# samxuxiang/BrepGen

Measured on NVIDIA H100. Metric: B-reps/sec (1000-step ABC cascade), higher is better.
Workload: dtype f16 x f16 -> f32 (wgmma; split hi+lo weights on in/out-proj; fp32 residual/LN/softmax)

## Files before the change

brepgen_b200/csrc/gemm.cu:

```cuda
#include <stdlib.h>

#include "bg_internal.h"
#include "gemm_epilogue.cuh"
#include "ptx.cuh"

namespace bg {

namespace {

constexpr int BM = 128;
constexpr int BK = 64;

template <int BN>
struct Cfg {
  static constexpr int STAGES = (BN == 256) ? 4 : 6;
  static constexpr int A_BYTES = BM * BK * 2;
  static constexpr int B_BYTES = BN * BK * 2;
  static constexpr int STAGE_BYTES = A_BYTES + B_BYTES;
  static constexpr int BAR_BYTES = 256;
  static constexpr int SMEM_BYTES = STAGES * STAGE_BYTES + BAR_BYTES + 1024;
};

template <int BN>
__device__ __forceinline__ void wgmma_tile_k16(float (&acc)[BN / 2], uint64_t a, uint64_t b, uint32_t accumulate) {
  if constexpr (BN == 256) wgmma_m64n256k16_ss(acc, a, b, accumulate);
  else wgmma_m64n128k16_ss(acc, a, b, accumulate);
}

template <int BN>
__global__ void __launch_bounds__(384, 1)
gemm_f16_kernel(const __grid_constant__ CUtensorMap tmA, const __grid_constant__ CUtensorMap tmB, const GemmParams p_in) {
  const GemmParams p = gemm_resolve(p_in);
  using C = Cfg<BN>;
  extern __shared__ uint8_t smem_raw[];
  uint8_t* smem = reinterpret_cast<uint8_t*>((reinterpret_cast<uintptr_t>(smem_raw) + 1023) & ~uintptr_t(1023));
  uint64_t* full = reinterpret_cast<uint64_t*>(smem + C::STAGES * C::STAGE_BYTES);
  uint64_t* empty = full + C::STAGES;

  const int warp = threadIdx.x >> 5;
  const int lane = threadIdx.x & 31;
  const int wg = threadIdx.x >> 7;

  if (threadIdx.x == 0) {
    tma_prefetch_desc(&tmA);
    tma_prefetch_desc(&tmB);
    for (int i = 0; i < C::STAGES; ++i) {
      mbar_init(&full[i], 1);
      mbar_init(&empty[i], 256);
    }
    fence_barrier_init();
  }
  __syncthreads();

  const int num_m = (p.M + BM - 1) / BM;
  const int num_n = p.N / BN;
  const int num_tiles = num_m * num_n;
  const int num_k = p.K / BK;

  if (wg == 0) {
    setmaxnreg_dec<40>();
    if (warp == 0 && elect_one()) {
      int stage = 0;
      uint32_t phase = 0;
      for (int tile = blockIdx.x; tile < num_tiles; tile += gridDim.x) {
        const int m_blk = tile / num_n, n_blk = tile % num_n;
        const int nk = (n_blk * BN < p.n_short) ? p.k_short / BK : num_k;
        gemm_prefetch_resid<BM, BN>(p, m_blk * BM, n_blk * BN);
        for (int kb = 0; kb < nk; ++kb) {
          mbar_wait(&empty[stage], phase ^ 1);
          uint8_t* sA = smem + stage * C::STAGE_BYTES;
          uint8_t* sB = sA + C::A_BYTES;
          mbar_arrive_expect_tx(&full[stage], C::STAGE_BYTES);
          if (p.conv_taps) {
            int c0, x, y, n;
            conv_coords(p, kb, m_blk * BM, c0, x, y, n);
            tma_load_4d(sA, &tmA, &full[stage], c0, x, y, n);
          } else {
            const int ka = p.a_kwrap ? (kb * BK) % p.a_kwrap : kb * BK;
            tma_load_2d(sA, &tmA, &full[stage], ka, m_blk * BM);
          }
          tma_load_2d(sB, &tmB, &full[stage], kb * BK, n_blk * BN);
          if (++stage == C::STAGES) { stage = 0; phase ^= 1; }
        }
      }
    }
  } else {
    setmaxnreg_inc<232>();
    const int half = wg - 1;
    float acc[BN / 2];
    int stage = 0;
    uint32_t phase = 0;
    for (int tile = blockIdx.x; tile < num_tiles; tile += gridDim.x) {
      const int m_blk = tile / num_n, n_blk = tile % num_n;
      const int nk = (n_blk * BN < p.n_short) ? p.k_short / BK : num_k;
      int prev = -1;
      for (int kb = 0; kb < nk; ++kb) {
        mbar_wait(&full[stage], phase);
        const uint32_t a_addr = smem_u32(smem + stage * C::STAGE_BYTES) + half * 64 * 128;
        const uint32_t b_addr = smem_u32(smem + stage * C::STAGE_BYTES + C::A_BYTES);
        wgmma_fence_operand(acc);
        wgmma_fence();
#pragma unroll
        for (int k = 0; k < BK / 16; ++k)
          wgmma_tile_k16<BN>(acc, make_sw128_desc(a_addr + k * 32), make_sw128_desc(b_addr + k * 32), (kb | k) != 0 ? 1u : 0u);
        wgmma_commit();
        wgmma_fence_operand(acc);
        wgmma_wait<1>();
        if (prev >= 0) mbar_arrive(&empty[prev]);
        prev = stage;
        if (++stage == C::STAGES) { stage = 0; phase ^= 1; }
      }
      wgmma_wait<0>();
      wgmma_fence_operand(acc);
      mbar_arrive(&empty[prev]);
      gemm_epilogue_regs<BN>(p, acc, m_blk * BM + half * 64, n_blk * BN, warp & 3, lane);
    }
  }
}

template <int BN>
int launch_bn(cudaStream_t st, const CUtensorMap& tmA, const CUtensorMap& tmB, const GemmParams& p) {
  using C = Cfg<BN>;
  BG_TRY(ensure_dynamic_smem(reinterpret_cast<const void*>(&gemm_f16_kernel<BN>), C::SMEM_BYTES));
  const int num_tiles = ((p.M + BM - 1) / BM) * (p.N / BN);
  const int grid = num_tiles < num_sms() ? num_tiles : num_sms();
  gemm_f16_kernel<BN><<<grid, 384, C::SMEM_BYTES, st>>>(tmA, tmB, p);
  return check_launch("gemm_f16_kernel launch");
}

namespace pp {
constexpr int BN = 128;
constexpr int STAGES = 5;
constexpr int STAGE_BYTES = (BM + BN) * BK * 2;
constexpr int BOX_BYTES = BM * 128;
constexpr int STAGING_BYTES = BM * BN * 4;
constexpr int BAR_BYTES = 256;
constexpr int SMEM_BYTES = STAGES * STAGE_BYTES + STAGING_BYTES + BAR_BYTES + 1024;
}

__device__ __forceinline__ void pp_advance(int& stage, uint32_t& phase, int n) {
  stage += n;
  while (stage >= pp::STAGES) { stage -= pp::STAGES; phase ^= 1; }
}

__device__ __forceinline__ void pp_arm_staging(const GemmParams& p, const CUtensorMap* tmR, uint8_t* stg, uint64_t* bar,
                                               int tile, int num_n) {
  if (p.resid) {
    const int row0 = (tile / num_n) * BM, col0 = (tile % num_n) * pp::BN;
    mbar_arrive_expect_tx(bar, pp::STAGING_BYTES);
#pragma unroll
    for (int b = 0; b < 4; ++b) tma_load_2d(stg + b * pp::BOX_BYTES, tmR, bar, col0 + 32 * b, row0);
  } else {
    mbar_arrive(bar);
  }
}

__device__ __forceinline__ void pp_epilogue_smem(const GemmParams& p, const float (&acc)[2][64], uint8_t* stg, int col0,
                                                 int warp_in_wg, int lane) {
  const int q = lane & 3;
#pragma unroll
  for (int i = 0; i < pp::BN / 8; ++i) {
    float2 b = make_float2(0.f, 0.f);
    if (p.bias) b = __ldg(reinterpret_cast<const float2*>(p.bias + col0 + 8 * i + 2 * q));
#pragma unroll
    for (int h = 0; h < 2; ++h) {
#pragma unroll
      for (int hr = 0; hr < 2; ++hr) {
        const int r = h * 64 + warp_in_wg * 16 + hr * 8 + (lane >> 2);
        float v0 = acc[h][4 * i + 2 * hr], v1 = acc[h][4 * i + 2 * hr + 1];
        if (p.bias) {
          v0 += b.x;
          v1 += b.y;
        }
        float2* d = reinterpret_cast<float2*>(stg + (i >> 2) * pp::BOX_BYTES + r * 128 +
                                              (((2 * (i & 3) + (q >> 1)) ^ (r & 7)) << 4) + 8 * (q & 1));
        if (p.resid) {
          const float2 rr = *d;
          v0 += rr.x;
          v1 += rr.y;
        }
        if (p.relu) {
          v0 = fmaxf(v0, 0.f);
          v1 = fmaxf(v1, 0.f);
        }
        *d = make_float2(v0, v1);
      }
    }
  }
}

__global__ void __launch_bounds__(384, 1)
gemm_pp_kernel(const __grid_constant__ CUtensorMap tmA, const __grid_constant__ CUtensorMap tmB,
               const __grid_constant__ CUtensorMap tmO, const __grid_constant__ CUtensorMap tmR, const GemmParams p_in) {
  const GemmParams p = gemm_resolve(p_in);
  extern __shared__ uint8_t smem_raw[];
  uint8_t* smem = reinterpret_cast<uint8_t*>((reinterpret_cast<uintptr_t>(smem_raw) + 1023) & ~uintptr_t(1023));
  uint8_t* stg = smem + pp::STAGES * pp::STAGE_BYTES;
  uint64_t* full = reinterpret_cast<uint64_t*>(stg + pp::STAGING_BYTES);
  uint64_t* empty = full + pp::STAGES;
  uint64_t* turn = empty + pp::STAGES;
  uint64_t* ready = turn + 2;

  const int warp = threadIdx.x >> 5;
  const int lane = threadIdx.x & 31;
  const int wg = threadIdx.x >> 7;

  const int num_m = (p.M + BM - 1) / BM;
  const int num_n = p.N / pp::BN;
  const int num_tiles = num_m * num_n;
  const int num_k = p.K / BK;

  if (threadIdx.x == 0) {
    tma_prefetch_desc(&tmA);
    tma_prefetch_desc(&tmB);
    tma_prefetch_desc(&tmO);
    for (int i = 0; i < pp::STAGES; ++i) {
      mbar_init(&full[i], 1);
      mbar_init(&empty[i], 128);
    }
    for (int c = 0; c < 2; ++c) {
      mbar_init(&turn[c], 128);
      mbar_init(&ready[c], 1);
    }
    fence_barrier_init();
  }
  __syncthreads();
  if (threadIdx.x == 0 && (int)blockIdx.x < num_tiles) pp_arm_staging(p, &tmR, stg, &ready[0], blockIdx.x, num_n);

  if (wg == 0) {
    setmaxnreg_dec<40>();
    if (warp == 0 && elect_one()) {
      int stage = 0;
      uint32_t phase = 0;
      for (int tile = blockIdx.x; tile < num_tiles; tile += gridDim.x) {
        const int m_blk = tile / num_n, n_blk = tile % num_n;
        const int nk = (n_blk * pp::BN < p.n_short) ? p.k_short / BK : num_k;
        for (int kb = 0; kb < nk; ++kb) {
          mbar_wait(&empty[stage], phase ^ 1);
          uint8_t* sA = smem + stage * pp::STAGE_BYTES;
          uint8_t* sB = sA + BM * BK * 2;
          mbar_arrive_expect_tx(&full[stage], pp::STAGE_BYTES);
          const int ka = p.a_kwrap ? (kb * BK) % p.a_kwrap : kb * BK;
          tma_load_2d(sA, &tmA, &full[stage], ka, m_blk * BM);
          tma_load_2d(sB, &tmB, &full[stage], kb * BK, n_blk * pp::BN);
          pp_advance(stage, phase, 1);
        }
      }
    }
  } else {
    setmaxnreg_inc<232>();
    const int c = wg - 1;
    float acc[2][64];
    int stage = 0;
    uint32_t phase = 0;
    int j = 0;
    for (int t = 0, tile = blockIdx.x; tile < num_tiles; ++t, tile += gridDim.x) {
      const int m_blk = tile / num_n, n_blk = tile % num_n;
      const int nk = (n_blk * pp::BN < p.n_short) ? p.k_short / BK : num_k;
      if ((t & 1) != c) {
        pp_advance(stage, phase, nk);
        continue;
      }
      if (t > 0) mbar_wait(&turn[c], ((t - 1) >> 1) & 1);
      int prev = -1;
      for (int kb = 0; kb < nk; ++kb) {
        mbar_wait(&full[stage], phase);
        const uint32_t a_addr = smem_u32(smem + stage * pp::STAGE_BYTES);
        const uint32_t b_addr = a_addr + BM * BK * 2;
        wgmma_fence_operand(acc[0]);
        wgmma_fence_operand(acc[1]);
        wgmma_fence();
#pragma unroll
        for (int k = 0; k < BK / 16; ++k) {
          const uint64_t bd = make_sw128_desc(b_addr + k * 32);
          wgmma_m64n128k16_ss(acc[0], make_sw128_desc(a_addr + k * 32), bd, (kb | k) != 0 ? 1u : 0u);
          wgmma_m64n128k16_ss(acc[1], make_sw128_desc(a_addr + 64 * 128 + k * 32), bd, (kb | k) != 0 ? 1u : 0u);
        }
        wgmma_commit();
        wgmma_fence_operand(acc[0]);
        wgmma_fence_operand(acc[1]);
        wgmma_wait<1>();
        if (prev >= 0) mbar_arrive(&empty[prev]);
        prev = stage;
        pp_advance(stage, phase, 1);
      }
      mbar_arrive(&turn[c ^ 1]);
      wgmma_wait<0>();
      wgmma_fence_operand(acc[0]);
      wgmma_fence_operand(acc[1]);
      mbar_arrive(&empty[prev]);

      const int row0 = m_blk * BM, col0 = n_blk * pp::BN;
      mbar_wait(&ready[c], j & 1);
      const bool leader = (threadIdx.x & 127) == 0;
      if (row0 + BM <= p.M) {
        pp_epilogue_smem(p, acc, stg, col0, warp & 3, lane);
        fence_proxy_async_shared();
        named_bar_sync(1 + c, 128);
        if (leader) {
          for (int b = 0; b < 4; ++b) tma_store_2d(&tmO, stg + b * pp::BOX_BYTES, col0 + 32 * b, row0);
          bulk_commit();
          bulk_wait_read_all();
        }
      } else {
        gemm_epilogue_regs<pp::BN>(p, acc[0], row0, col0, warp & 3, lane);
        gemm_epilogue_regs<pp::BN>(p, acc[1], row0 + 64, col0, warp & 3, lane);
      }
      if (leader && tile + (int)gridDim.x < num_tiles)
        pp_arm_staging(p, &tmR, stg, &ready[c ^ 1], tile + gridDim.x, num_n);
      ++j;
    }
  }
}

int launch_pp(cudaStream_t st, const CUtensorMap& tmA, const CUtensorMap& tmB, const CUtensorMap& tmO,
              const CUtensorMap& tmR, const GemmParams& p) {
  BG_TRY(ensure_dynamic_smem(reinterpret_cast<const void*>(&gemm_pp_kernel), pp::SMEM_BYTES));
  const int num_tiles = ((p.M + BM - 1) / BM) * (p.N / pp::BN);
  const int grid = num_tiles < num_sms() ? num_tiles : num_sms();
  gemm_pp_kernel<<<grid, 384, pp::SMEM_BYTES, st>>>(tmA, tmB, tmO, tmR, p);
  return check_launch("gemm_pp_kernel launch");
}

bool pingpong_enabled() {
  static const bool on = [] {
    const char* e = getenv("BREPGEN_B200_GEMM_PINGPONG");
    return !(e && atoi(e) == 0);
  }();
  return on;
}

}

int launch_gemm_f16(cudaStream_t st, const __half* A, int lda, const __half* W, int ldw, int M, int N, int K,
                    const GemmEpilogue& ep) {
  BG_REQUIRE(M > 0 && N > 0 && K > 0, "gemm: empty problem");
  BG_REQUIRE(K % BK == 0, "gemm: K must be a multiple of 64");
  BG_REQUIRE(N % 128 == 0, "gemm: N must be a multiple of 128");
  BG_REQUIRE(lda % 8 == 0 && ldw % 8 == 0, "gemm: operand pitch must be a multiple of 8 elements (16 B)");
  BG_REQUIRE((reinterpret_cast<uintptr_t>(A) & 15) == 0 && (reinterpret_cast<uintptr_t>(W) & 15) == 0,
             "gemm: operands must be 16-byte aligned");
  BG_REQUIRE(ep.out != nullptr && ep.ldo % 8 == 0, "gemm: output pitch must be a multiple of 8");
  BG_REQUIRE((reinterpret_cast<uintptr_t>(ep.out) & 15) == 0, "gemm: output must be 16-byte aligned");
  BG_REQUIRE(ep.resid == nullptr || (ep.ldr % 4 == 0 && !ep.out_f16 ? true : ep.ldr % 4 == 0), "gemm: resid pitch");
  BG_REQUIRE(ep.rowvec == nullptr || (ep.rows_per_vec > 0 && ep.ldv % 4 == 0), "gemm: rowvec");
  BG_REQUIRE(!ep.out_f16 || (ep.resid == nullptr && ep.rowvec == nullptr), "gemm: fp16 output supports bias / ReLU only");
  BG_REQUIRE((reinterpret_cast<uintptr_t>(ep.bias) & 7) == 0, "gemm: bias must be 8-byte aligned");
  BG_REQUIRE((reinterpret_cast<uintptr_t>(ep.resid) & 7) == 0, "gemm: resid must be 8-byte aligned");
  int bn = (N % 256 == 0) ? 256 : 128;
  if (bn == 256 && (long long)((M + BM - 1) / BM) * (N / 256) < num_sms()) bn = 128;
  const bool use_pp = pingpong_enabled() && !ep.out_f16 && ep.conv.taps == 0 && ep.rowvec == nullptr &&
                      ep.row_map == nullptr && (reinterpret_cast<uintptr_t>(ep.resid) & 15) == 0;
  if (use_pp) bn = pp::BN;
  CUtensorMap tmA, tmB;
  const int a_cols = ep.a_kwrap > 0 ? ep.a_kwrap : K;
  BG_REQUIRE(ep.a_kwrap == 0 || (ep.a_kwrap % BK == 0 && ep.a_kwrap <= K), "gemm: a_kwrap must be a multiple of 64");
  const ConvGeom& cg = ep.conv;
  if (cg.taps > 0) {
    const int hw = cg.W * cg.H;
    BG_REQUIRE(cg.C > 0 && cg.C % 64 == 0 && cg.W > 0 && cg.H > 0 && cg.N > 0 && cg.kw > 0 && cg.taps % cg.kw == 0,
               "conv gemm: bad geometry");
    BG_REQUIRE(128 % cg.W == 0 && (hw % 128 == 0 || 128 % hw == 0), "conv gemm: W * H must divide 128 or be a multiple of it");
    BG_REQUIRE(M == cg.N * hw && K == cg.terms * cg.taps * cg.C && ep.a_kwrap == 0, "conv gemm: M / K do not match the geometry");
    BG_REQUIRE(lda >= (cg.lo_plane ? 2 : 1) * cg.C, "conv gemm: channel pitch too small");
    const int box_h = hw >= 128 ? 128 / cg.W : cg.H, box_n = hw >= 128 ? 1 : 128 / hw;
    BG_TRY(make_tmap_4d_f16(&tmA, A, (uint64_t)(cg.lo_plane ? 2 : 1) * cg.C, cg.W, cg.H, cg.N, (uint64_t)lda, cg.W, box_h, box_n));
  } else {
    BG_TRY(make_tmap_2d_f16(&tmA, A, (uint64_t)M, (uint64_t)a_cols, (uint64_t)lda, BM));
  }
  BG_TRY(make_tmap_2d_f16(&tmB, W, (uint64_t)N, (uint64_t)K, (uint64_t)ldw, (uint32_t)bn));
  GemmParams p;
  p.M = M; p.N = N; p.K = K; p.a_kwrap = ep.a_kwrap; p.m_dev = ep.m_dev; p.row_map = ep.row_map;
  p.n_short = ep.n_short; p.k_short = ep.k_short;
  BG_REQUIRE(ep.n_short == 0 || (ep.n_short % 256 == 0 && ep.k_short % BK == 0 && ep.k_short > 0 && ep.k_short <= K),
             "gemm: n_short must be a multiple of 256 and k_short a multiple of 64");
  p.out = ep.out; p.ldo = ep.ldo; p.out_f16 = ep.out_f16; p.relu = ep.relu;
  p.bias = ep.bias; p.resid = ep.resid; p.ldr = ep.ldr;
  p.rowvec = ep.rowvec; p.rows_per_vec = ep.rows_per_vec; p.ldv = ep.ldv;
  p.conv_taps = cg.taps; p.conv_kw = cg.kw; p.conv_cpb = cg.C / 64; p.conv_C = cg.C; p.conv_W = cg.W; p.conv_HW = cg.W * cg.H;
  p.conv_pad_w = cg.kw / 2; p.conv_pad_h = cg.taps > 0 ? (cg.taps / cg.kw) / 2 : 0;
  p.conv_lo_term = (cg.taps > 0 && cg.lo_plane && cg.terms == 3) ? 1 : -1;
  if (use_pp) {
    CUtensorMap tmO, tmR;
    BG_TRY(make_tmap_2d_f32(&tmO, ep.out, (uint64_t)M, (uint64_t)N, (uint64_t)ep.ldo, BM, 32));
    tmR = tmO;
    if (ep.resid) BG_TRY(make_tmap_2d_f32(&tmR, ep.resid, (uint64_t)M, (uint64_t)N, (uint64_t)ep.ldr, BM, 32));
    return launch_pp(st, tmA, tmB, tmO, tmR, p);
  }
  return bn == 256 ? launch_bn<256>(st, tmA, tmB, p) : launch_bn<128>(st, tmA, tmB, p);
}

}
```

brepgen_b200/csrc/ptx.cuh:

```cuda
#pragma once
#include <cuda.h>
#include <cuda_fp16.h>
#include <cuda_runtime.h>
#include <stdint.h>

namespace bg {

__device__ __forceinline__ uint32_t smem_u32(const void* p) { return (uint32_t)__cvta_generic_to_shared(p); }

__device__ __forceinline__ bool elect_one() {
  uint32_t pred;
  asm volatile(
      "{\n\t.reg .pred P;\n\t.reg .b32 R;\n\t"
      "elect.sync R|P, 0xffffffff;\n\t"
      "selp.b32 %0, 1, 0, P;\n\t}\n"
      : "=r"(pred));
  return pred != 0;
}

__device__ __forceinline__ void mbar_init(uint64_t* bar, uint32_t count) {
  asm volatile("mbarrier.init.shared::cta.b64 [%0], %1;" ::"r"(smem_u32(bar)), "r"(count));
}
__device__ __forceinline__ void fence_barrier_init() { asm volatile("fence.mbarrier_init.release.cluster;" ::: "memory"); }
__device__ __forceinline__ void mbar_arrive(uint64_t* bar) {
  asm volatile("mbarrier.arrive.shared::cta.b64 _, [%0];" ::"r"(smem_u32(bar)) : "memory");
}
__device__ __forceinline__ void mbar_arrive_expect_tx(uint64_t* bar, uint32_t bytes) {
  asm volatile("mbarrier.arrive.expect_tx.shared::cta.b64 _, [%0], %1;" ::"r"(smem_u32(bar)), "r"(bytes) : "memory");
}
__device__ __forceinline__ bool mbar_try_wait(uint64_t* bar, uint32_t parity) {
  uint32_t ok;
  asm volatile(
      "{\n\t.reg .pred P;\n\t"
      "mbarrier.try_wait.parity.shared::cta.b64 P, [%1], %2;\n\t"
      "selp.b32 %0, 1, 0, P;\n\t}\n"
      : "=r"(ok)
      : "r"(smem_u32(bar)), "r"(parity)
      : "memory");
  return ok != 0;
}
__device__ __forceinline__ void mbar_wait(uint64_t* bar, uint32_t parity) {
  uint32_t spins = 0;
  while (!mbar_try_wait(bar, parity)) {
    if (++spins > (1u << 26)) asm volatile("trap;");
  }
}

__device__ __forceinline__ void tma_prefetch_desc(const CUtensorMap* m) {
  asm volatile("prefetch.tensormap [%0];" ::"l"(reinterpret_cast<uint64_t>(m)) : "memory");
}
__device__ __forceinline__ void tma_load_2d(void* smem_dst, const CUtensorMap* m, uint64_t* bar, int c0, int c1) {
  asm volatile(
      "cp.async.bulk.tensor.2d.shared::cluster.global.mbarrier::complete_tx::bytes [%0], [%1, {%3, %4}], [%2];"
      ::"r"(smem_u32(smem_dst)), "l"(reinterpret_cast<uint64_t>(m)), "r"(smem_u32(bar)), "r"(c0), "r"(c1)
      : "memory");
}

__device__ __forceinline__ void tma_load_4d(void* smem_dst, const CUtensorMap* m, uint64_t* bar, int c0, int c1, int c2, int c3) {
  asm volatile(
      "cp.async.bulk.tensor.4d.shared::cluster.global.mbarrier::complete_tx::bytes [%0], [%1, {%3, %4, %5, %6}], [%2];"
      ::"r"(smem_u32(smem_dst)), "l"(reinterpret_cast<uint64_t>(m)), "r"(smem_u32(bar)), "r"(c0), "r"(c1), "r"(c2), "r"(c3)
      : "memory");
}

__device__ __forceinline__ void tma_store_2d(const CUtensorMap* m, const void* smem_src, int c0, int c1) {
  asm volatile("cp.async.bulk.tensor.2d.global.shared::cta.bulk_group [%0, {%2, %3}], [%1];"
               ::"l"(reinterpret_cast<uint64_t>(m)), "r"(smem_u32(smem_src)), "r"(c0), "r"(c1)
               : "memory");
}
__device__ __forceinline__ void bulk_commit() { asm volatile("cp.async.bulk.commit_group;" ::: "memory"); }
__device__ __forceinline__ void bulk_wait_read_all() { asm volatile("cp.async.bulk.wait_group.read 0;" ::: "memory"); }
__device__ __forceinline__ void fence_proxy_async_shared() { asm volatile("fence.proxy.async.shared::cta;" ::: "memory"); }
__device__ __forceinline__ void named_bar_sync(uint32_t id, uint32_t count) {
  asm volatile("bar.sync %0, %1;" ::"r"(id), "r"(count) : "memory");
}

__device__ __forceinline__ void prefetch_l2_bulk(const void* p, uint32_t bytes) {
  asm volatile("cp.async.bulk.prefetch.L2.global [%0], %1;" ::"l"(reinterpret_cast<uint64_t>(p)), "r"(bytes) : "memory");
}

template <uint32_t N>
__device__ __forceinline__ void setmaxnreg_dec() { asm volatile("setmaxnreg.dec.sync.aligned.u32 %0;" ::"n"(N)); }
template <uint32_t N>
__device__ __forceinline__ void setmaxnreg_inc() { asm volatile("setmaxnreg.inc.sync.aligned.u32 %0;" ::"n"(N)); }

__device__ __forceinline__ uint64_t make_sw128_desc(uint32_t smem_addr, uint32_t sbo_bytes = 1024) {
  uint64_t d = 0;
  d |= (uint64_t)((smem_addr & 0x3FFFF) >> 4);
  d |= (uint64_t)1 << 16;
  d |= (uint64_t)((sbo_bytes >> 4) & 0x3FFF) << 32;
  d |= (uint64_t)1 << 62;
  return d;
}

__device__ __forceinline__ void wgmma_fence() { asm volatile("wgmma.fence.sync.aligned;" ::: "memory"); }
__device__ __forceinline__ void wgmma_commit() { asm volatile("wgmma.commit_group.sync.aligned;" ::: "memory"); }
template <int N>
__device__ __forceinline__ void wgmma_wait() { asm volatile("wgmma.wait_group.sync.aligned %0;" ::"n"(N) : "memory"); }
template <int R>
__device__ __forceinline__ void wgmma_fence_operand(float (&d)[R]) {
#pragma unroll
  for (int i = 0; i < R; ++i) asm volatile("" : "+f"(d[i])::"memory");
}

__device__ __forceinline__ void wgmma_m64n256k16_ss(float (&d)[128], uint64_t a_desc, uint64_t b_desc, uint32_t accumulate) {
  asm volatile(
      "{\n\t.reg .pred p;\n\t"
      "setp.ne.b32 p, %130, 0;\n\t"
      "wgmma.mma_async.sync.aligned.m64n256k16.f32.f16.f16 "
      "{%0, %1, %2, %3, %4, %5, %6, %7, %8, %9, %10, %11, %12, %13, %14, %15, "
      "%16, %17, %18, %19, %20, %21, %22, %23, %24, %25, %26, %27, %28, %29, %30, %31, "
      "%32, %33, %34, %35, %36, %37, %38, %39, %40, %41, %42, %43, %44, %45, %46, %47, "
      "%48, %49, %50, %51, %52, %53, %54, %55, %56, %57, %58, %59, %60, %61, %62, %63, "
      "%64, %65, %66, %67, %68, %69, %70, %71, %72, %73, %74, %75, %76, %77, %78, %79, "
      "%80, %81, %82, %83, %84, %85, %86, %87, %88, %89, %90, %91, %92, %93, %94, %95, "
      "%96, %97, %98, %99, %100, %101, %102, %103, %104, %105, %106, %107, %108, %109, %110, %111, "
      "%112, %113, %114, %115, %116, %117, %118, %119, %120, %121, %122, %123, %124, %125, %126, %127}, "
      "%128, %129, p, 1, 1, 0, 0;\n\t}\n"
      : "+f"(d[0]), "+f"(d[1]), "+f"(d[2]), "+f"(d[3]), "+f"(d[4]), "+f"(d[5]), "+f"(d[6]), "+f"(d[7]),
        "+f"(d[8]), "+f"(d[9]), "+f"(d[10]), "+f"(d[11]), "+f"(d[12]), "+f"(d[13]), "+f"(d[14]), "+f"(d[15]),
        "+f"(d[16]), "+f"(d[17]), "+f"(d[18]), "+f"(d[19]), "+f"(d[20]), "+f"(d[21]), "+f"(d[22]), "+f"(d[23]),
        "+f"(d[24]), "+f"(d[25]), "+f"(d[26]), "+f"(d[27]), "+f"(d[28]), "+f"(d[29]), "+f"(d[30]), "+f"(d[31]),
        "+f"(d[32]), "+f"(d[33]), "+f"(d[34]), "+f"(d[35]), "+f"(d[36]), "+f"(d[37]), "+f"(d[38]), "+f"(d[39]),
        "+f"(d[40]), "+f"(d[41]), "+f"(d[42]), "+f"(d[43]), "+f"(d[44]), "+f"(d[45]), "+f"(d[46]), "+f"(d[47]),
        "+f"(d[48]), "+f"(d[49]), "+f"(d[50]), "+f"(d[51]), "+f"(d[52]), "+f"(d[53]), "+f"(d[54]), "+f"(d[55]),
        "+f"(d[56]), "+f"(d[57]), "+f"(d[58]), "+f"(d[59]), "+f"(d[60]), "+f"(d[61]), "+f"(d[62]), "+f"(d[63]),
        "+f"(d[64]), "+f"(d[65]), "+f"(d[66]), "+f"(d[67]), "+f"(d[68]), "+f"(d[69]), "+f"(d[70]), "+f"(d[71]),
        "+f"(d[72]), "+f"(d[73]), "+f"(d[74]), "+f"(d[75]), "+f"(d[76]), "+f"(d[77]), "+f"(d[78]), "+f"(d[79]),
        "+f"(d[80]), "+f"(d[81]), "+f"(d[82]), "+f"(d[83]), "+f"(d[84]), "+f"(d[85]), "+f"(d[86]), "+f"(d[87]),
        "+f"(d[88]), "+f"(d[89]), "+f"(d[90]), "+f"(d[91]), "+f"(d[92]), "+f"(d[93]), "+f"(d[94]), "+f"(d[95]),
        "+f"(d[96]), "+f"(d[97]), "+f"(d[98]), "+f"(d[99]), "+f"(d[100]), "+f"(d[101]), "+f"(d[102]), "+f"(d[103]),
        "+f"(d[104]), "+f"(d[105]), "+f"(d[106]), "+f"(d[107]), "+f"(d[108]), "+f"(d[109]), "+f"(d[110]), "+f"(d[111]),
        "+f"(d[112]), "+f"(d[113]), "+f"(d[114]), "+f"(d[115]), "+f"(d[116]), "+f"(d[117]), "+f"(d[118]), "+f"(d[119]),
        "+f"(d[120]), "+f"(d[121]), "+f"(d[122]), "+f"(d[123]), "+f"(d[124]), "+f"(d[125]), "+f"(d[126]), "+f"(d[127])
      : "l"(a_desc), "l"(b_desc), "r"(accumulate));
}

__device__ __forceinline__ void wgmma_m64n128k16_ss(float (&d)[64], uint64_t a_desc, uint64_t b_desc, uint32_t accumulate) {
  asm volatile(
      "{\n\t.reg .pred p;\n\t"
      "setp.ne.b32 p, %66, 0;\n\t"
      "wgmma.mma_async.sync.aligned.m64n128k16.f32.f16.f16 "
      "{%0, %1, %2, %3, %4, %5, %6, %7, %8, %9, %10, %11, %12, %13, %14, %15, "
      "%16, %17, %18, %19, %20, %21, %22, %23, %24, %25, %26, %27, %28, %29, %30, %31, "
      "%32, %33, %34, %35, %36, %37, %38, %39, %40, %41, %42, %43, %44, %45, %46, %47, "
      "%48, %49, %50, %51, %52, %53, %54, %55, %56, %57, %58, %59, %60, %61, %62, %63}, "
      "%64, %65, p, 1, 1, 0, 0;\n\t}\n"
      : "+f"(d[0]), "+f"(d[1]), "+f"(d[2]), "+f"(d[3]), "+f"(d[4]), "+f"(d[5]), "+f"(d[6]), "+f"(d[7]),
        "+f"(d[8]), "+f"(d[9]), "+f"(d[10]), "+f"(d[11]), "+f"(d[12]), "+f"(d[13]), "+f"(d[14]), "+f"(d[15]),
        "+f"(d[16]), "+f"(d[17]), "+f"(d[18]), "+f"(d[19]), "+f"(d[20]), "+f"(d[21]), "+f"(d[22]), "+f"(d[23]),
        "+f"(d[24]), "+f"(d[25]), "+f"(d[26]), "+f"(d[27]), "+f"(d[28]), "+f"(d[29]), "+f"(d[30]), "+f"(d[31]),
        "+f"(d[32]), "+f"(d[33]), "+f"(d[34]), "+f"(d[35]), "+f"(d[36]), "+f"(d[37]), "+f"(d[38]), "+f"(d[39]),
        "+f"(d[40]), "+f"(d[41]), "+f"(d[42]), "+f"(d[43]), "+f"(d[44]), "+f"(d[45]), "+f"(d[46]), "+f"(d[47]),
        "+f"(d[48]), "+f"(d[49]), "+f"(d[50]), "+f"(d[51]), "+f"(d[52]), "+f"(d[53]), "+f"(d[54]), "+f"(d[55]),
        "+f"(d[56]), "+f"(d[57]), "+f"(d[58]), "+f"(d[59]), "+f"(d[60]), "+f"(d[61]), "+f"(d[62]), "+f"(d[63])
      : "l"(a_desc), "l"(b_desc), "r"(accumulate));
}

__device__ __forceinline__ void wgmma_m64n64k16_rs_bt(float (&d)[32], const uint32_t (&a)[4], uint64_t b_desc, uint32_t accumulate) {
  asm volatile(
      "{\n\t.reg .pred p;\n\t"
      "setp.ne.b32 p, %37, 0;\n\t"
      "wgmma.mma_async.sync.aligned.m64n64k16.f32.f16.f16 "
      "{%0, %1, %2, %3, %4, %5, %6, %7, %8, %9, %10, %11, %12, %13, %14, %15, "
      "%16, %17, %18, %19, %20, %21, %22, %23, %24, %25, %26, %27, %28, %29, %30, %31}, "
      "{%32, %33, %34, %35}, %36, p, 1, 1, 1;\n\t}\n"
      : "+f"(d[0]), "+f"(d[1]), "+f"(d[2]), "+f"(d[3]), "+f"(d[4]), "+f"(d[5]), "+f"(d[6]), "+f"(d[7]),
        "+f"(d[8]), "+f"(d[9]), "+f"(d[10]), "+f"(d[11]), "+f"(d[12]), "+f"(d[13]), "+f"(d[14]), "+f"(d[15]),
        "+f"(d[16]), "+f"(d[17]), "+f"(d[18]), "+f"(d[19]), "+f"(d[20]), "+f"(d[21]), "+f"(d[22]), "+f"(d[23]),
        "+f"(d[24]), "+f"(d[25]), "+f"(d[26]), "+f"(d[27]), "+f"(d[28]), "+f"(d[29]), "+f"(d[30]), "+f"(d[31])
      : "r"(a[0]), "r"(a[1]), "r"(a[2]), "r"(a[3]), "l"(b_desc), "r"(accumulate));
}


__device__ __forceinline__ float ex2(float x) {
  float y;
  asm("ex2.approx.ftz.f32 %0, %1;" : "=f"(y) : "f"(x));
  return y;
}

__device__ __forceinline__ uint32_t pack_half2(float a, float b) {
  __half2 h = __floats2half2_rn(a, b);
  return *reinterpret_cast<uint32_t*>(&h);
}

}
```

Baseline: 0.1905.

## Stage f16 GEMM epilogue through swizzled smem and store with TMA

For BN=256 GEMMs with f16 output and no conv taps, the epilogue now applies bias and ReLU in registers, writes packed half2 values into a 128B-swizzled shared staging buffer, and issues TMA 2D bulk stores instead of scattered register stores to global memory. Partial M tiles fall back to vectorized 16-byte copies out of the staging buffer. The aim is coalesced, asynchronous output writes that overlap with the next tile's mainloop. In exchange the pipeline drops from 4 to 3 stages to make room for the staging buffer, which may expose more load latency.

```diff
diff --git a/brepgen_b200/csrc/gemm.cu b/brepgen_b200/csrc/gemm.cu
--- a/brepgen_b200/csrc/gemm.cu
+++ b/brepgen_b200/csrc/gemm.cu
@@ -11,14 +11,16 @@
 constexpr int BM = 128;
 constexpr int BK = 64;
 
-template <int BN>
+template <int BN, bool STAGED>
 struct Cfg {
-  static constexpr int STAGES = (BN == 256) ? 4 : 6;
+  static constexpr int STAGES = STAGED ? 3 : (BN == 256) ? 4 : 6;
   static constexpr int A_BYTES = BM * BK * 2;
   static constexpr int B_BYTES = BN * BK * 2;
   static constexpr int STAGE_BYTES = A_BYTES + B_BYTES;
+  static constexpr int BOX_BYTES = 64 * 128;
+  static constexpr int STAGING_BYTES = STAGED ? BM * BN * 2 : 0;
   static constexpr int BAR_BYTES = 256;
-  static constexpr int SMEM_BYTES = STAGES * STAGE_BYTES + BAR_BYTES + 1024;
+  static constexpr int SMEM_BYTES = STAGES * STAGE_BYTES + STAGING_BYTES + BAR_BYTES + 1024;
 };
 
 template <int BN>
@@ -27,14 +29,59 @@
   else wgmma_m64n128k16_ss(acc, a, b, accumulate);
 }
 
+template <int BN, bool BIAS, bool RELU>
+__device__ __forceinline__ void f16_epilogue_smem(const GemmParams& p, const float (&acc)[BN / 2], uint32_t stg, int col0,
+                                                  int warp_in_wg, int lane) {
+  const int q = lane & 3;
+  const float2* bias = reinterpret_cast<const float2*>(p.bias + col0 + 2 * q);
+  const uint32_t row_base = stg + (warp_in_wg * 16 + (lane >> 2)) * 128 + ((lane >> 2) << 4) + 4 * q;
+#pragma unroll
+  for (int j = 0; j < 8; ++j) {
+    const uint32_t chunk = row_base ^ (j << 4);
+#pragma unroll
+    for (int box = 0; box < BN / 64; ++box) {
+      const int i = 8 * box + j;
+      float2 b;
+      if (BIAS) b = __ldg(bias + 4 * i);
+#pragma unroll
+      for (int hr = 0; hr < 2; ++hr) {
+        float v0 = acc[4 * i + 2 * hr], v1 = acc[4 * i + 2 * hr + 1];
+        if (BIAS) {
+          v0 += b.x;
+          v1 += b.y;
+        }
+        if (RELU) {
+          v0 = fmaxf(v0, 0.f);
+          v1 = fmaxf(v1, 0.f);
+        }
+        st_shared_u32(chunk + box * Cfg<BN, true>::BOX_BYTES + hr * 8 * 128, pack_half2(v0, v1));
+      }
+    }
+  }
+}
+
 template <int BN>
+__device__ __forceinline__ void f16_epilogue_smem(const GemmParams& p, const float (&acc)[BN / 2], uint32_t stg, int col0,
+                                                  int warp_in_wg, int lane) {
+  if (p.bias) {
+    if (p.relu) f16_epilogue_smem<BN, true, true>(p, acc, stg, col0, warp_in_wg, lane);
+    else f16_epilogue_smem<BN, true, false>(p, acc, stg, col0, warp_in_wg, lane);
+  } else {
+    if (p.relu) f16_epilogue_smem<BN, false, true>(p, acc, stg, col0, warp_in_wg, lane);
+    else f16_epilogue_smem<BN, false, false>(p, acc, stg, col0, warp_in_wg, lane);
+  }
+}
+
+template <int BN, bool STAGED>
 __global__ void __launch_bounds__(384, 1)
-gemm_f16_kernel(const __grid_constant__ CUtensorMap tmA, const __grid_constant__ CUtensorMap tmB, const GemmParams p_in) {
+gemm_f16_kernel(const __grid_constant__ CUtensorMap tmA, const __grid_constant__ CUtensorMap tmB,
+                const __grid_constant__ CUtensorMap tmO, const GemmParams p_in) {
   const GemmParams p = gemm_resolve(p_in);
-  using C = Cfg<BN>;
+  using C = Cfg<BN, STAGED>;
   extern __shared__ uint8_t smem_raw[];
   uint8_t* smem = reinterpret_cast<uint8_t*>((reinterpret_cast<uintptr_t>(smem_raw) + 1023) & ~uintptr_t(1023));
-  uint64_t* full = reinterpret_cast<uint64_t*>(smem + C::STAGES * C::STAGE_BYTES);
+  uint8_t* stg = smem + C::STAGES * C::STAGE_BYTES;
+  uint64_t* full = reinterpret_cast<uint64_t*>(stg + C::STAGING_BYTES);
   uint64_t* empty = full + C::STAGES;
 
   const int warp = threadIdx.x >> 5;
@@ -44,6 +91,7 @@
   if (threadIdx.x == 0) {
     tma_prefetch_desc(&tmA);
     tma_prefetch_desc(&tmB);
+    if (STAGED) tma_prefetch_desc(&tmO);
     for (int i = 0; i < C::STAGES; ++i) {
       mbar_init(&full[i], 1);
       mbar_init(&empty[i], 256);
@@ -113,18 +161,45 @@
       wgmma_wait<0>();
       wgmma_fence_operand(acc);
       mbar_arrive(&empty[prev]);
-      gemm_epilogue_regs<BN>(p, acc, m_blk * BM + half * 64, n_blk * BN, warp & 3, lane);
-    }
-  }
-}
-
-template <int BN>
-int launch_bn(cudaStream_t st, const CUtensorMap& tmA, const CUtensorMap& tmB, const GemmParams& p) {
-  using C = Cfg<BN>;
-  BG_TRY(ensure_dynamic_smem(reinterpret_cast<const void*>(&gemm_f16_kernel<BN>), C::SMEM_BYTES));
+      const int row0 = m_blk * BM + half * 64, col0 = n_blk * BN;
+      if (STAGED) {
+        uint8_t* half_stg = stg + half * (C::STAGING_BYTES / 2);
+        const bool leader = (threadIdx.x & 127) == 0;
+        if (leader) bulk_wait_read_all();
+        named_bar_sync(1 + half, 128);
+        f16_epilogue_smem<BN>(p, acc, smem_u32(half_stg), col0, warp & 3, lane);
+        fence_proxy_async_shared();
+        named_bar_sync(1 + half, 128);
+        if (m_blk * BM + BM <= p.M) {
+          if (leader) {
+#pragma unroll
+            for (int b = 0; b < BN / 64; ++b) tma_store_2d(&tmO, half_stg + b * C::BOX_BYTES, col0 + 64 * b, row0);
+            bulk_commit();
+          }
+        } else {
+          for (int c = threadIdx.x & 127; c < 64 * (BN / 8); c += 128) {
+            const int r = c / (BN / 8), g = c % (BN / 8);
+            if (row0 + r >= p.M) break;
+            const uint4 v = *reinterpret_cast<const uint4*>(half_stg + (g >> 3) * C::BOX_BYTES + r * 128 +
+                                                             (((g & 7) ^ (r & 7)) << 4));
+            *reinterpret_cast<uint4*>(reinterpret_cast<__half*>(p.out) + (size_t)(row0 + r) * p.ldo + col0 + 8 * g) = v;
+          }
+        }
+      } else {
+        gemm_epilogue_regs<BN>(p, acc, row0, col0, warp & 3, lane);
+      }
+    }
+    if (STAGED && (threadIdx.x & 127) == 0) bulk_wait_read_all();
+  }
+}
+
+template <int BN, bool STAGED>
+int launch_bn(cudaStream_t st, const CUtensorMap& tmA, const CUtensorMap& tmB, const CUtensorMap& tmO, const GemmParams& p) {
+  using C = Cfg<BN, STAGED>;
+  BG_TRY(ensure_dynamic_smem(reinterpret_cast<const void*>(&gemm_f16_kernel<BN, STAGED>), C::SMEM_BYTES));
   const int num_tiles = ((p.M + BM - 1) / BM) * (p.N / BN);
   const int grid = num_tiles < num_sms() ? num_tiles : num_sms();
-  gemm_f16_kernel<BN><<<grid, 384, C::SMEM_BYTES, st>>>(tmA, tmB, p);
+  gemm_f16_kernel<BN, STAGED><<<grid, 384, C::SMEM_BYTES, st>>>(tmA, tmB, tmO, p);
   return check_launch("gemm_f16_kernel launch");
 }
 
@@ -387,7 +462,13 @@
     if (ep.resid) BG_TRY(make_tmap_2d_f32(&tmR, ep.resid, (uint64_t)M, (uint64_t)N, (uint64_t)ep.ldr, BM, 32));
     return launch_pp(st, tmA, tmB, tmO, tmR, p);
   }
-  return bn == 256 ? launch_bn<256>(st, tmA, tmB, p) : launch_bn<128>(st, tmA, tmB, p);
-}
-
-}
+  if (bn == 256 && ep.out_f16 && cg.taps == 0 && pingpong_enabled()) {
+    CUtensorMap tmO;
+    BG_TRY(make_tmap_2d_f16(&tmO, ep.out, (uint64_t)M, (uint64_t)N, (uint64_t)ep.ldo, 64, 64));
+    return launch_bn<256, true>(st, tmA, tmB, tmO, p);
+  }
+  return bn == 256 ? launch_bn<256, false>(st, tmA, tmB, tmA , p)
+                   : launch_bn<128, false>(st, tmA, tmB, tmA , p);
+}
+
+}
diff --git a/brepgen_b200/csrc/ptx.cuh b/brepgen_b200/csrc/ptx.cuh
--- a/brepgen_b200/csrc/ptx.cuh
+++ b/brepgen_b200/csrc/ptx.cuh
@@ -71,6 +71,9 @@
 __device__ __forceinline__ void bulk_commit() { asm volatile("cp.async.bulk.commit_group;" ::: "memory"); }
 __device__ __forceinline__ void bulk_wait_read_all() { asm volatile("cp.async.bulk.wait_group.read 0;" ::: "memory"); }
 __device__ __forceinline__ void fence_proxy_async_shared() { asm volatile("fence.proxy.async.shared::cta;" ::: "memory"); }
+__device__ __forceinline__ void st_shared_u32(uint32_t addr, uint32_t v) {
+  asm volatile("st.shared.b32 [%0], %1;" ::"r"(addr), "r"(v) : "memory");
+}
 __device__ __forceinline__ void named_bar_sync(uint32_t id, uint32_t count) {
   asm volatile("bar.sync %0, %1;" ::"r"(id), "r"(count) : "memory");
 }
```

Measured after the change: 0.1947 (median of 6 runs). 2.2% higher.
